# rlawhdrhs/Vision-Transformer-OpenCL

Hardware: AMD Instinct MI355X
Metric: images/sec ViT-B/16 224² fp32 @batch256; % MFMA roofline; top-1 match (higher is better)
Workload: dtype f32; 1 GPU; ViT-B/16 224x224 fp32 forward, batch 256 per GPU, synthetic weights and images (BASELINE.json configs[1]); batch_per_gpu=256, global_batch=256, parallelism=dp1, lanes_per_gpu=1, prune_last_layer=False, ln_fold=True, device=AMD Radeon Graphics, arch=gfx950:sramecc+:xnack-, compute_units=256, clock_mhz=2400

## Files before the change

### include/vit_hip_kernels.h

```cpp
#ifndef VIT_HIP_KERNELS_H
#define VIT_HIP_KERNELS_H

#include <stddef.h>

#ifdef __cplusplus
extern "C" {
#endif

typedef void *vithip_stream_t;
typedef void *vithip_event_t;
typedef void *vithip_graph_t;

typedef struct {
    char name[256];
    char arch[64];
    int compute_units;
    int clock_mhz;
    int wavefront;
    int lds_per_block;
    unsigned long long hbm_bytes;
} vithip_device_info;

const char *vithip_error_string(int code);
int vithip_device_count(int *count);
// ... 81 lines not shown
int vithip_gemm_bf16(vithip_stream_t stream, const vithip_gemm_bf16_args *args);
int vithip_ln_fold_weights(vithip_stream_t stream, const float *W, const float *bias, const float *gamma, const float *beta,
                           unsigned short *Wf, float *colsum, float *bias_f, int N, int K);
#define VITHIP_QSCALE 0.18033688011112042f
int vithip_ln_fold_weights_scaled(vithip_stream_t stream, const float *W, const float *bias, const float *gamma, const float *beta,
                                  unsigned short *Wf, float *colsum, float *bias_f, int N, int K, int scale_rows, float scale);
int vithip_rowstats_bf16(vithip_stream_t stream, const float *x, size_t ldx, unsigned short *x16, size_t ldx16,
                         float *rows_out, int rows, int dim);
int vithip_rowstats_bf16_eps(vithip_stream_t stream, const float *x, size_t ldx, unsigned short *x16, size_t ldx16,
                             float *rows_out, int rows, int dim, double eps);
int vithip_ln_strips(int N);
int vithip_rowstats_finalize(vithip_stream_t stream, const float *partials, int strips, int rows, int dim, float *rows_out);
int vithip_rowstats_finalize_eps(vithip_stream_t stream, const float *partials, int strips, int rows, int dim, float *rows_out, double eps);
int vithip_gather_rows_f32(vithip_stream_t stream, const float *src, size_t src_stride, float *dst, size_t dst_stride, int rows,
                           int width);
int vithip_layernorm_f32_bf16out(vithip_stream_t stream, const float *x, size_t ldx, unsigned short *y, size_t ldy,
                                 const float *gamma, const float *beta, int rows, int dim);
int vithip_layernorm_f32_bf16out_eps(vithip_stream_t stream, const float *x, size_t ldx, unsigned short *y, size_t ldy,
                                     const float *gamma, const float *beta, int rows, int dim, double eps);
int vithip_attention_bf16io(vithip_stream_t stream, const unsigned short *qkv, unsigned short *out,
                            int n_images, int tokens, int heads);
int vithip_attention_bf16io_f32math(vithip_stream_t stream, const unsigned short *qkv, unsigned short *out,
                                    int n_images, int tokens, int heads);
int vithip_attention_f32_rows(vithip_stream_t stream, const float *qkv, float *out, int n_images, int tokens, int heads,
                              int q_rows);
int vithip_attention_bf16io_rows(vithip_stream_t stream, const unsigned short *qkv, unsigned short *out, int n_images,
                                 int tokens, int heads, int q_rows);
int vithip_attention_bf16io_qscaled(vithip_stream_t stream, const unsigned short *qkv, unsigned short *out, int n_images,
                                    int tokens, int heads, int q_rows);
int vithip_attention_f32_hd(vithip_stream_t stream, const float *qkv, float *out, int n_images, int tokens, int heads, int head_dim,
                            int q_rows);
int vithip_attention_bf16io_hd(vithip_stream_t stream, const unsigned short *qkv, unsigned short *out, int n_images, int tokens,
                               int heads, int head_dim, int q_rows, int q_scaled);
float vithip_qscale(int head_dim);
int vithip_patch_embed_bf16(vithip_stream_t stream, const float *images, const unsigned short *conv_w16,
                            const float *conv_b, const float *cls, const float *pos, float *x,
                            unsigned short *patches16, int n_images, int img_size, int patch_size, int in_chans,
                            int embed_dim);
int vithip_patch_embed_bf16_implicit(vithip_stream_t stream, const float *images, const unsigned short *conv_w16,
                                     const float *conv_b, const float *cls, const float *pos, float *x,
                                     int n_images, int img_size, int patch_size, int in_chans, int embed_dim);
int vithip_f32_to_bf16(vithip_stream_t stream, const float *src, unsigned short *dst, size_t count);

int vithip_patch_embed_f32(vithip_stream_t stream, const float *images, const float *conv_w,
                           const float *conv_b, const float *cls, const float *pos, float *x,
                           int n_images, int img_size, int patch_size, int in_chans, int embed_dim);
int vithip_patch_embed_f32_general(vithip_stream_t stream, const float *images, const float *conv_w,
                                   const float *conv_b, const float *cls, const float *pos, float *x,
                                   int n_images, int img_size, int patch_size, int in_chans, int embed_dim);

int vithip_layernorm_f32(vithip_stream_t stream, const float *x, size_t ldx, float *y, size_t ldy,
                         const float *gamma, const float *beta, int rows, int dim);
int vithip_layernorm_f32_eps(vithip_stream_t stream, const float *x, size_t ldx, float *y, size_t ldy,
                             const float *gamma, const float *beta, int rows, int dim, double eps);

int vithip_swiglu_f32(vithip_stream_t stream, const float *u, size_t ldu, float *h, size_t ldh, int rows, int H);
int vithip_swiglu_bf16(vithip_stream_t stream, const unsigned short *u, size_t ldu, unsigned short *h, size_t ldh, int rows, int H);

int vithip_attention_f32(vithip_stream_t stream, const float *qkv, float *out,
                         int n_images, int tokens, int heads);

int vithip_softmax_top1_f32(vithip_stream_t stream, const float *logits, int ld_logits,
                            float *probs, int ld_probs, int *top1_label, float *top1_prob,
                            int rows, int classes);

enum { VITHIP_SCORE_PROB = 0, VITHIP_SCORE_LOGIT = 1 };
// ... 59 lines not shown
```

### vision-transformer-opencl_amd/binding.py

```python
from __future__ import annotations

import ctypes as C
import os
from typing import Optional, Sequence

import numpy as np

from .synth import MLP_CODES, MLP_SHIFT, ModelConfig

HERE = os.path.dirname(os.path.abspath(__file__))
LIB_PATH = os.environ.get("VIT_HIP_LIBRARY") or os.path.join(HERE, "libvit_mi355x.so")

f32p = C.POINTER(C.c_float)
i32p = C.POINTER(C.c_int)

STAGES = ("embed", "ln", "qkv", "attn", "outproj", "fc1", "fc2", "head", "softmax")
IMAGENET_MEAN = (0.485, 0.456, 0.406)
IMAGENET_STD = (0.229, 0.224, 0.225)
EPI_BIAS, EPI_BIAS_GELU, EPI_BIAS_RESIDUAL = 0, 1, 2
EPI_BIAS_QGELU = 6
ARITH_F32, ARITH_SPLIT3 = 0, 1


class VitError(RuntimeError):
# ... 305 lines not shown
        L.vit_argmax.argtypes = [f32p, C.c_int]
        L.ViT_hip.argtypes = [C.POINTER(CImageData), C.POINTER(CNetwork), C.POINTER(f32p)]
        L.ViT_opencl.argtypes = [C.POINTER(CImageData), C.POINTER(CNetwork), C.POINTER(f32p)]
        for fn in ("vithip_malloc", "vithip_host_alloc"):
            getattr(L, fn).argtypes = [C.POINTER(C.c_void_p), C.c_size_t]
        L.vithip_free.argtypes = [C.c_void_p]
        for fn in ("vithip_memcpy_h2d", "vithip_memcpy_d2h", "vithip_memcpy_d2d"):
            getattr(L, fn).argtypes = [C.c_void_p, C.c_void_p, C.c_size_t, C.c_void_p]
        L.vithip_gemm_f32.argtypes = [C.c_void_p, C.POINTER(CGemmArgs)]
        L.vithip_split3_weights_bytes.argtypes = [C.c_int, C.c_int]
        L.vithip_split3_weights_bytes.restype = C.c_size_t
        L.vithip_split3_weights_f32.argtypes = [C.c_void_p, C.c_void_p, C.c_int, C.c_int, C.c_int, C.c_void_p]
        L.vithip_patch_embed_f32.argtypes = [C.c_void_p] + [C.c_void_p] * 6 + [C.c_int] * 5
        if hasattr(L, "vithip_patch_embed_f32_general"):
            L.vithip_patch_embed_f32_general.argtypes = [C.c_void_p] + [C.c_void_p] * 6 + [C.c_int] * 5
            L.vit_weights_fold_layer_scale.argtypes = [C.POINTER(CConfig), C.POINTER(CNetwork), C.c_int, C.POINTER(CNetwork), C.c_int]
        L.vithip_layernorm_f32.argtypes = [C.c_void_p, C.c_void_p, C.c_size_t, C.c_void_p, C.c_size_t,
                                           C.c_void_p, C.c_void_p, C.c_int, C.c_int]
        pv, cls = [C.c_void_p] * 3, [C.c_void_p, C.c_void_p, C.c_size_t, C.c_void_p, C.c_size_t]
        for fn in ("vithip_attention_f32", "vithip_attention_bf16io", "vithip_attention_bf16io_f32math"):
            getattr(L, fn).argtypes = pv + [C.c_int] * 3
        for fn in ("vithip_attention_f32_rows", "vithip_attention_bf16io_rows", "vithip_attention_bf16io_qscaled"):
            getattr(L, fn).argtypes = pv + [C.c_int] * 4
        if hasattr(L, "vit_engine_cls_attention_device"):
            L.vithip_cls_attention_f32.argtypes = cls + [C.c_int] * 4
            L.vithip_cls_attention_bf16.argtypes = cls + [C.c_int] * 5
        if hasattr(L, "vithip_attention_f32_hd"):
            L.vithip_qscale.restype = C.c_float
            L.vithip_qscale.argtypes = [C.c_int]
            L.vithip_attention_f32_hd.argtypes = pv + [C.c_int] * 5
            L.vithip_attention_bf16io_hd.argtypes = pv + [C.c_int] * 6
            L.vithip_cls_attention_f32_hd.argtypes = cls + [C.c_int] * 5
            L.vithip_cls_attention_bf16_hd.argtypes = cls + [C.c_int] * 6
        L.vithip_softmax_top1_f32.argtypes = [C.c_void_p, C.c_void_p, C.c_int, C.c_void_p, C.c_int, C.c_void_p,
                                              C.c_void_p, C.c_int, C.c_int]
        L.vithip_event_create.argtypes = [C.POINTER(C.c_void_p)]
        L.vithip_event_record.argtypes = [C.c_void_p, C.c_void_p]
        L.vithip_event_sync.argtypes = [C.c_void_p]
        L.vithip_event_destroy.argtypes = [C.c_void_p]
        L.vithip_event_elapsed_ms.argtypes = [C.POINTER(C.c_float), C.c_void_p, C.c_void_p]
        L.vithip_stream_sync.argtypes = [C.c_void_p]
        L.vithip_get_device_info.argtypes = [C.c_int, C.POINTER(CDeviceInfo)]
        _lib = L
    return _lib


def hip_check(rc: int, what: str = "HIP call") -> None:
    if rc != 0:
        err = VitError(f"{what}: HIP error {rc} ({lib().vithip_error_string(rc).decode()})")
        err.code = int(rc)
        raise err


def _as_f32(a) -> np.ndarray:
    return np.ascontiguousarray(a, dtype=np.float32)


def networks_from(weights: Sequence[np.ndarray]):
    arr = (CNetwork * len(weights))()
    keep = []
    for i, w in enumerate(weights):
        if w is None:
            arr[i].data = None
            arr[i].size = 0
        else:
            w = _as_f32(w)
# ... 526 lines not shown
    _note(out, dst=dd)
    hip_check(L.vithip_gather_rows_f32(None, None if null == "src" else ds.ptr, ds.ld if src_stride is None else src_stride,
                                       None if null == "dst" else dd.ptr, dd.ld if dst_stride is None else dst_stride,
                                       src.shape[0] if rows is None else rows, src.shape[1] if width is None else width),
              "vithip_gather_rows_f32")
    return dd.window()


def attention(qkv, n_images: int, tokens: int, heads: int) -> np.ndarray:
    return _attention("vithip_attention_f32", _as_f32(qkv), n_images, tokens, heads, 64, ())


def attention_rows(qkv, n_images: int, tokens: int, heads: int, q_rows: int, fill: float = 0.0, frames=None,
                   out: Optional[dict] = None) -> np.ndarray:
    return _attention("vithip_attention_f32_rows", _as_f32(qkv), n_images, tokens, heads, 64, (q_rows,), fill, frames, out)


def attention_bf16io_rows(qkv_bits, n_images: int, tokens: int, heads: int, q_rows: int, q_scaled: bool = False, frames=None,
                          out: Optional[dict] = None) -> np.ndarray:
    name = "vithip_attention_bf16io_qscaled" if q_scaled else "vithip_attention_bf16io_rows"
    return _attention(name, _bits(qkv_bits), n_images, tokens, heads, 64, (q_rows,), 0, frames, out)


def qscale(head_dim: int) -> float:
    return float(lib().vithip_qscale(int(head_dim)))


def attention_hd(qkv, n_images: int, tokens: int, heads: int, head_dim: int, q_rows: Optional[int] = None, fill: float = 0.0,
                 frames=None, out: Optional[dict] = None) -> np.ndarray:
    return _attention("vithip_attention_f32_hd", _as_f32(qkv), n_images, tokens, heads, head_dim,
                      (head_dim, tokens if q_rows is None else q_rows), fill, frames, out)


def attention_bf16io_hd(qkv_bits, n_images: int, tokens: int, heads: int, head_dim: int, q_rows: Optional[int] = None,
                        q_scaled: bool = False, fill: int = 0, frames=None, out: Optional[dict] = None) -> np.ndarray:
    return _attention("vithip_attention_bf16io_hd", _bits(qkv_bits), n_images, tokens, heads, head_dim,
                      (head_dim, tokens if q_rows is None else q_rows, int(q_scaled)), fill, frames, out)


def _cls_attention(name, qkv, n_images, tokens, heads, head_dim, head_mean, q_scaled, ld_out, fill):
    assert qkv.shape == (n_images * tokens, 3 * heads * head_dim)
    args = ((head_dim,) if name.endswith("_hd") else ()) + (int(head_mean),) + (() if q_scaled is None else (int(q_scaled),))
    row = tokens if head_mean else heads * tokens
    ld = row if ld_out is None else int(ld_out)
    do = DeviceArray((n_images, ld)) if fill is None else DeviceArray.from_numpy(np.full((n_images, ld), fill, np.float32))
    dq = DeviceArray.from_numpy(qkv)
    hip_check(getattr(lib(), name)(None, dq.ptr, 3 * heads * head_dim, do.ptr, ld, n_images, tokens, heads, *args), name)
    res = do.numpy()
    if ld_out is not None:
        return res
    return res if head_mean else res.reshape(n_images, heads, tokens)


def cls_attention(qkv, n_images: int, tokens: int, heads: int, head_mean: bool = False, ld_out: Optional[int] = None,
                  fill: Optional[float] = None) -> np.ndarray:
    return _cls_attention("vithip_cls_attention_f32", _as_f32(qkv), n_images, tokens, heads, 64, head_mean, None, ld_out, fill)


def cls_attention_bf16(qkv_bits, n_images: int, tokens: int, heads: int, head_mean: bool = False, q_scaled: bool = False,
                       ld_out: Optional[int] = None, fill: Optional[float] = None) -> np.ndarray:
    return _cls_attention("vithip_cls_attention_bf16", _bits(qkv_bits), n_images, tokens, heads, 64, head_mean, q_scaled, ld_out, fill)


def cls_attention_hd(qkv, n_images: int, tokens: int, heads: int, head_dim: int, head_mean: bool = False, ld_out: Optional[int] = None,
                     fill: Optional[float] = None) -> np.ndarray:
    return _cls_attention("vithip_cls_attention_f32_hd", _as_f32(qkv), n_images, tokens, heads, head_dim, head_mean, None, ld_out, fill)
# ... 738 lines not shown
```

### vision-transformer-opencl_amd/csrc/vit_attention.hip

```cpp
#include <hip/hip_runtime.h>

#include <type_traits>

#include "vit_attention.hpp"
#include "vit_device.hpp"
#include "vit_hip_kernels.h"
#ifdef VIT_PROBES
#include "vit_probes.h"
#endif

namespace {

using namespace vitattn;

template <typename IO> __device__ __forceinline__ f32x4 load4(const IO *p);
template <> __device__ __forceinline__ f32x4 load4<float>(const float *p) { return *reinterpret_cast<const f32x4 *>(p); }
template <> __device__ __forceinline__ f32x4 load4<bf16_t>(const bf16_t *p) {
    const uint2 b = *reinterpret_cast<const uint2 *>(p);
    f32x4 v;
    v[0] = __uint_as_float(b.x << 16);
    v[1] = __uint_as_float(b.x & 0xffff0000u);
    v[2] = __uint_as_float(b.y << 16);
    v[3] = __uint_as_float(b.y & 0xffff0000u);
    return v;
// ... 667 lines not shown
    hipLaunchKernelGGL(attention_bf16_kernel<NKT>, dim3(grid), dim3(ATT_THREADS), 0, s, qkv, out, tokens, heads, items, q_rows,
                       q_scaled ? 1.0f : kScale64);
    return static_cast<int>(hipGetLastError());
}

template <int NKT, typename IO>
int launch_f32(hipStream_t s, const IO *qkv, IO *out, int n_images, int tokens, int heads, int q_rows) {
    hipLaunchKernelGGL((attention_f32_kernel<NKT, IO>), dim3(heads, n_images), dim3(ATT_THREADS), 0, s, qkv, out,
                       tokens, heads, q_rows, g_attn_dbg);
    return static_cast<int>(hipGetLastError());
}

inline dim3 chunked_grid(int n_images, int tokens, int heads) {
    return dim3(heads, n_images, ((tokens + 31) / 32 + ATT_WAVES - 1) / ATT_WAVES);
}

template <typename IO>
int route_f32_math(hipStream_t s, const IO *qkv, IO *out, int n_images, int tokens, int heads, int q_rows) {
    if constexpr (std::is_same<IO, float>::value) {
        if (tokens <= 224) return attention_f32_resident(s, qkv, out, n_images, tokens, heads, q_rows);
    }
    if (tokens > 224) {
        hipLaunchKernelGGL(attention_f32_chunked_kernel<IO>, chunked_grid(n_images, tokens, heads), dim3(ATT_THREADS), 0, s, qkv, out,
                           tokens, heads);
        return static_cast<int>(hipGetLastError());
    }
    return dispatch_int<1, 7>((tokens + 31) / 32, [&](auto nkt) {
        return launch_f32<decltype(nkt)::value, IO>(s, qkv, out, n_images, tokens, heads, q_rows);
    });
}

template <typename IO>
int route(vithip_stream_t stream, const IO *qkv, IO *out, int n_images, int tokens, int heads, int head_dim, int q_rows, int q_scaled,
          bool f32_math = false, bool resident_only = false) {
    constexpr int refused = static_cast<int>(hipErrorInvalidValue);
    hipStream_t s = static_cast<hipStream_t>(stream);
    if (!hd_accepted(head_dim) || (q_scaled != 0 && q_scaled != 1) || !qkv_args_ok(qkv, out, n_images, tokens, heads, q_rows))
        return refused;
    if constexpr (std::is_same<IO, float>::value) {
        if (head_dim != 64) return attention_hd_f32(s, qkv, out, n_images, tokens, heads, head_dim, q_rows);
        if (tokens > 224 && (resident_only || q_rows < tokens)) return refused;
        return route_f32_math<float>(s, qkv, out, n_images, tokens, heads, q_rows);
    } else {
        if (head_dim != 64) return attention_hd_bf16(s, qkv, out, n_images, tokens, heads, head_dim, q_rows, q_scaled != 0);
        if (tokens > 224 && (resident_only || q_rows < tokens)) return refused;
        if (f32_math) return q_scaled ? refused : route_f32_math<bf16_t>(s, qkv, out, n_images, tokens, heads, q_rows);
        if (tokens <= 224)
            return dispatch_int<1, 7>((tokens + 31) / 32, [&](auto nkt) {
                return launch_bf16<decltype(nkt)::value>(s, qkv, out, n_images, tokens, heads, q_rows, q_scaled != 0);
            });
        if (tokens <= 704) return attention_bf16_stream(s, qkv, out, n_images, tokens, heads, q_scaled != 0);
        hipLaunchKernelGGL(attention_bf16_chunked_kernel, chunked_grid(n_images, tokens, heads), dim3(ATT_THREADS), 0, s, qkv, out, tokens,
                           heads, q_scaled ? 1.0f : kScale64);
        return static_cast<int>(hipGetLastError());
    }
}

}

#ifdef VIT_PROBES
extern "C" int vithip_attention_set_probe_mode(int mode) {
    vitattn::g_res_mode = mode;
    return 0;
}
extern "C" int vithip_attention_set_debug_buffer(void *buf) {
    g_attn_dbg = static_cast<unsigned long long *>(buf);
    vitattn::g_res_dbg = g_attn_dbg;
    vitattn::g_stream_dbg = g_attn_dbg;
    return 0;
}
#endif

extern "C" {


int vithip_attention_f32(vithip_stream_t stream, const float *qkv, float *out, int n_images, int tokens, int heads) {
    return route<float>(stream, qkv, out, n_images, tokens, heads, 64, tokens, 0);
}

int vithip_attention_f32_rows(vithip_stream_t stream, const float *qkv, float *out, int n_images, int tokens, int heads, int q_rows) {
    return route<float>(stream, qkv, out, n_images, tokens, heads, 64, q_rows, 0, false, true);
}

int vithip_attention_f32_hd(vithip_stream_t stream, const float *qkv, float *out, int n_images, int tokens, int heads, int head_dim,
                            int q_rows) {
    return route<float>(stream, qkv, out, n_images, tokens, heads, head_dim, q_rows, 0);
}

int vithip_attention_bf16io(vithip_stream_t stream, const unsigned short *qkv, unsigned short *out, int n_images, int tokens,
                            int heads) {
    return route<bf16_t>(stream, qkv, out, n_images, tokens, heads, 64, tokens, 0);
}

int vithip_attention_bf16io_rows(vithip_stream_t stream, const unsigned short *qkv, unsigned short *out, int n_images, int tokens,
                                 int heads, int q_rows) {
    return route<bf16_t>(stream, qkv, out, n_images, tokens, heads, 64, q_rows, 0, false, true);
}

int vithip_attention_bf16io_qscaled(vithip_stream_t stream, const unsigned short *qkv, unsigned short *out, int n_images, int tokens,
                                    int heads, int q_rows) {
    return route<bf16_t>(stream, qkv, out, n_images, tokens, heads, 64, q_rows, 1);
}

int vithip_attention_bf16io_f32math(vithip_stream_t stream, const unsigned short *qkv, unsigned short *out, int n_images, int tokens,
                                    int heads) {
    return route<bf16_t>(stream, qkv, out, n_images, tokens, heads, 64, tokens, 0, true);
}

int vithip_attention_bf16io_hd(vithip_stream_t stream, const unsigned short *qkv, unsigned short *out, int n_images, int tokens,
                               int heads, int head_dim, int q_rows, int q_scaled) {
    return route<bf16_t>(stream, qkv, out, n_images, tokens, heads, head_dim, q_rows, q_scaled);
}

}
```

### vision-transformer-opencl_amd/csrc/vit_attention.hpp

```cpp
#ifndef VIT_ATTENTION_HPP
#define VIT_ATTENTION_HPP

#include <hip/hip_runtime.h>

#include <type_traits>

#include "vit_hip_kernels.h"

namespace vitattn {

typedef float f32x4 __attribute__((ext_vector_type(4)));
typedef float f32x16 __attribute__((ext_vector_type(16)));
typedef unsigned short bf16_t;
typedef __attribute__((ext_vector_type(4))) __bf16 bf16x4;
typedef __attribute__((ext_vector_type(8))) __bf16 bf16x8;
typedef unsigned u32x4 __attribute__((ext_vector_type(4)));
typedef short short4v __attribute__((ext_vector_type(4)));
typedef short short8v __attribute__((ext_vector_type(8)));
typedef __attribute__((address_space(3))) short4v lds_short4v;
typedef __attribute__((address_space(3))) void lds_void;

constexpr float kScale64 = 0.125f * 1.4426950408889634f;
static_assert(kScale64 == VITHIP_QSCALE, "the kernels' factor and the one the engine folds into the Q rows are the same bits");

// ... 4 lines not shown
    const int chunk = (dt * 4 + 2 * g2 + (pq >> 1)) ^ (4 * ((q >> 1) & 1));
    const bf16_t *ptr = Vs + row * LD + chunk * 8 + 4 * (pq & 1);
    const short4v lo = __builtin_amdgcn_ds_read_tr16_b64_v4i16((lds_short4v *)ptr);
    const short4v hi = __builtin_amdgcn_ds_read_tr16_b64_v4i16((lds_short4v *)(ptr + 8 * LD));
    const short8v both = __builtin_shufflevector(lo, hi, 0, 1, 2, 3, 4, 5, 6, 7);
    return __builtin_bit_cast(bf16x8, both);
}


static inline bool qkv_args_ok(const void *qkv, const void *out, int n_images, int tokens, int heads, int q_rows) {
    const size_t low_bits = (reinterpret_cast<size_t>(qkv) | reinterpret_cast<size_t>(out)) & 15;
    return qkv && out && !low_bits && n_images > 0 && tokens > 0 && heads > 0 && q_rows > 0 && q_rows <= tokens;
}

static inline bool hd_accepted(int head_dim) { return head_dim == 64 || (head_dim >= 72 && head_dim <= 128 && head_dim % 8 == 0); }

template <int FIRST, int COUNT, int STEP = 1, typename F>
static inline int dispatch_int(int n, F &&f) {
    if constexpr (COUNT == 0) {
        return static_cast<int>(hipErrorInvalidValue);
    } else {
        if (n == FIRST) return f(std::integral_constant<int, FIRST>{});
        return dispatch_int<FIRST + STEP, COUNT - 1, STEP>(n, f);
    }
}


int attention_f32_resident(hipStream_t s, const float *qkv, float *out, int n_images, int tokens, int heads, int q_rows);
int attention_bf16_stream(hipStream_t s, const unsigned short *qkv, unsigned short *out, int n_images, int tokens, int heads, bool q_scaled);
__attribute__((visibility("hidden"))) int attention_hd_f32(hipStream_t s, const float *qkv, float *out, int n_images, int tokens,
                                                           int heads, int head_dim, int q_rows);
__attribute__((visibility("hidden"))) int attention_hd_bf16(hipStream_t s, const unsigned short *qkv, unsigned short *out, int n_images,
                                                            int tokens, int heads, int head_dim, int q_rows, bool q_scaled);

#ifdef VIT_PROBES
extern unsigned long long *g_res_dbg;
extern int g_res_mode;
extern unsigned long long *g_stream_dbg;
#endif

}

#endif
```

### vision-transformer-opencl_amd/csrc/vit_attention_hd.hip

```cpp
#include <hip/hip_runtime.h>

#include <math.h>

#include <type_traits>

#include "vit_attention.hpp"
#include "vit_hip_kernels.h"

namespace {

using namespace vitattn;
typedef unsigned int u32x2 __attribute__((ext_vector_type(2)));

constexpr int HD_WAVES = 4, HD_THREADS = HD_WAVES * 64;
constexpr int HD_QROWS = HD_WAVES * 32;

template <int HD, bool BF16>
struct Geo {
    typedef typename std::conditional<BF16, bf16_t, float>::type elem;
    static constexpr int VEC = BF16 ? 8 : 4;
    static constexpr int KC = BF16 ? 64 : 32;
    static constexpr int KT = KC / 32;
    static constexpr int DT = (HD + 31) / 32;
    static constexpr int HDK = BF16 ? (HD + 15) / 16 * 16 : HD;
    static constexpr int KROW = HDK + (BF16 ? 8 : 4);
    static constexpr int VROW = KC + 4;
    static constexpr int K_ELEMS = KC * KROW, V_ELEMS = DT * 32 * VROW;
    static constexpr int MIN_WAVES = BF16 && HD <= 96 ? 4 : 3;
};

template <int HD, bool BF16, bool QS>
__global__ __launch_bounds__(HD_THREADS, (Geo<HD, BF16>::MIN_WAVES)) void attention_hd_kernel(
    const typename Geo<HD, BF16>::elem *__restrict__ qkv, typename Geo<HD, BF16>::elem *__restrict__ out, int tokens, int heads, int q_rows,
    int qblocks, float scale) {
    typedef Geo<HD, BF16> G;
    typedef typename G::elem elem;
    constexpr int VEC = G::VEC, KC = G::KC, KT = G::KT, DT = G::DT, KROW = G::KROW, VROW = G::VROW;
    __shared__ __attribute__((aligned(16))) elem Ks[G::K_ELEMS];
    __shared__ __attribute__((aligned(16))) elem Vt[G::V_ELEMS];

// ... 144 lines not shown
#pragma unroll
                            for (int i = 0; i < 4; ++i) o[dt] = __builtin_amdgcn_mfma_f32_32x32x2f32(vf[i], s[4 * q + i], o[dt], 0, 0, 0);
                        }
                }
            }
        }
        __syncthreads();
    }

    const int qrow = qrow0 + r;
    if (active && qrow < q_rows) {
        const float inv = 1.0f / (l_run + __shfl_xor(l_run, 32));
        elem *dst = out + ((size_t)image * tokens + qrow) * D + (size_t)head * HD;
#pragma unroll
        for (int dt = 0; dt < DT; ++dt)
#pragma unroll
            for (int q = 0; q < 4; ++q) {
                const int d0 = 32 * dt + 8 * q + 4 * h;
                if (d0 < HD) {
                    if constexpr (BF16) {
                        bf16x4 w;
#pragma unroll
                        for (int i = 0; i < 4; ++i) w[i] = (__bf16)(o[dt][4 * q + i] * inv);
                        *reinterpret_cast<u32x2 *>(dst + d0) = __builtin_bit_cast(u32x2, w);
                    } else {
                        const f32x4 w = {o[dt][4 * q] * inv, o[dt][4 * q + 1] * inv, o[dt][4 * q + 2] * inv, o[dt][4 * q + 3] * inv};
                        *reinterpret_cast<f32x4 *>(dst + d0) = w;
                    }
                }
            }
    }
}

template <bool BF16, bool QS>
int launch_hd(hipStream_t s, const typename Geo<128, BF16>::elem *qkv, typename Geo<128, BF16>::elem *out, int n_images, int tokens,
              int heads, int head_dim, int q_rows) {
    const int qblocks = (q_rows + HD_QROWS - 1) / HD_QROWS;
    if (heads > 65535 || (long long)n_images * qblocks > 0x7fffffffLL) return static_cast<int>(hipErrorInvalidValue);
    const float scale = QS ? 1.0f : vithip_qscale(head_dim);
    return dispatch_int<72, 8, 8>(head_dim, [&](auto hd) {
        hipLaunchKernelGGL((attention_hd_kernel<decltype(hd)::value, BF16, QS>), dim3((unsigned)(n_images * qblocks), (unsigned)heads),
                           dim3(HD_THREADS), 0, s, qkv, out, tokens, heads, q_rows, qblocks, scale);
        return static_cast<int>(hipGetLastError());
    });
}

}

int vitattn::attention_hd_f32(hipStream_t s, const float *qkv, float *out, int n_images, int tokens, int heads, int head_dim, int q_rows) {
    return launch_hd<false, false>(s, qkv, out, n_images, tokens, heads, head_dim, q_rows);
}

int vitattn::attention_hd_bf16(hipStream_t s, const unsigned short *qkv, unsigned short *out, int n_images, int tokens, int heads,
                               int head_dim, int q_rows, bool q_scaled) {
    return q_scaled ? launch_hd<true, true>(s, qkv, out, n_images, tokens, heads, head_dim, q_rows)
                    : launch_hd<true, false>(s, qkv, out, n_images, tokens, heads, head_dim, q_rows);
}

extern "C" float vithip_qscale(int head_dim) {
    if (!vitattn::hd_accepted(head_dim)) return 0.0f;
    return (float)((1.0 / sqrt((double)head_dim)) * 1.4426950408889634074);
}
```

### vision-transformer-opencl_amd/csrc/vit_gemm_common.hpp

```cpp
#pragma once
#include <hip/hip_runtime.h>

#include <type_traits>

#include "vit_hip_kernels.h"

namespace vitgemm {


typedef float f32x16 __attribute__((ext_vector_type(16)));
typedef float f32x4 __attribute__((ext_vector_type(4)));
typedef float f32x2 __attribute__((ext_vector_type(2)));
typedef unsigned u32x4 __attribute__((ext_vector_type(4)));

constexpr int KALIGN = 32;

enum { A_DENSE = 0, A_PATCHES = 1 };
enum { EPI_BIAS_LN = 3, EPI_BIAS_GELU_LN = 4, EPI_RESIDUAL_STATS = 5, EPI_BIAS_QGELU_LN = 7  };
constexpr bool epi_is_fold(int epi) { return epi == EPI_BIAS_LN || epi == EPI_BIAS_GELU_LN || epi == EPI_BIAS_QGELU_LN; }
constexpr bool epi_is_gelu(int epi) { return epi == VITHIP_EPI_BIAS_GELU || epi == EPI_BIAS_GELU_LN; }
constexpr bool epi_is_qgelu(int epi) { return epi == VITHIP_EPI_BIAS_QGELU || epi == EPI_BIAS_QGELU_LN; }

struct GemmParams {
    const float *A;
    const float *W;
    const float *bias;
    const float *R;
    float *C;
    int lda, ldw, ldr, ldc;
    int M, N, K;
    int tiles_m, tiles_n;
    int group_m;
    const float *pos;
    unsigned long long *dbg;
    int patches;
    int grid;
    int patch;
    int img;
// ... 130 lines not shown
}
__device__ __forceinline__ void quick_gelu_x8(float (&y)[8]) {
    f32x2 yy[4];
#pragma unroll
    for (int v = 0; v < 4; ++v) yy[v] = f32x2{y[2 * v], y[2 * v + 1]};
    quick_gelu_lockstep<4>(yy);
#pragma unroll
    for (int v = 0; v < 4; ++v) y[2 * v] = yy[v].x, y[2 * v + 1] = yy[v].y;
}

__device__ __forceinline__ int xcd_remap(int bid, int nwg) {
    const int q = nwg >> 3, rem = nwg & 7;
    const int xcd = bid & 7, idx = bid >> 3;
    const int base = xcd < rem ? xcd * (q + 1) : rem * (q + 1) + (xcd - rem) * q;
    return base + idx;
}

__device__ __forceinline__ void tile_coords(int tile, int tiles_m, int tiles_n, int group_m, int &tm, int &tn) {
    const int per_group = group_m * tiles_n;
    const int g = tile / per_group, in_g = tile - g * per_group;
    const int first = g * group_m;
    const int rows = tiles_m - first < group_m ? tiles_m - first : group_m;
    tn = in_g / rows;
    tm = first + (in_g - tn * rows);
}


enum { ARITH_F32 = 0, ARITH_SPLIT3 = 1 };
typedef __bf16 bf16x8 __attribute__((ext_vector_type(8)));
typedef __bf16 bf16x4 __attribute__((ext_vector_type(4)));
typedef unsigned u32x2 __attribute__((ext_vector_type(2)));
constexpr int SPLIT_BK = 16;
constexpr int SPLIT_LD = 28;
constexpr int SPLIT_TERM_A[6] = {0, 2, 1, 0, 1, 0};
constexpr int SPLIT_TERM_W[6] = {2, 0, 1, 1, 0, 0};

__device__ __forceinline__ float bf16_to_f32(__bf16 v) {
    return __builtin_bit_cast(float, (unsigned)__builtin_bit_cast(unsigned short, v) << 16);
}
__device__ __forceinline__ u32x2 split3_piece(f32x4 &x, int piece) {
    bf16x4 b;
#pragma unroll
    for (int e = 0; e < 4; ++e) b[e] = (__bf16)x[e];
    if (piece < 2) {
#pragma unroll
        for (int e = 0; e < 4; ++e) x[e] = x[e] - bf16_to_f32(b[e]);
    }
    return __builtin_bit_cast(u32x2, b);
}
__device__ __forceinline__ void split3_store(float *row, int kc, f32x4 x) {
#pragma unroll
    for (int piece = 0; piece < 3; ++piece) *reinterpret_cast<u32x2 *>(row + piece * 8 + kc / 2) = split3_piece(x, piece);
}
__device__ __forceinline__ u32x4 split3_piece8(f32x4 &x0, f32x4 &x1, int piece) {
    const u32x2 p0 = split3_piece(x0, piece), p1 = split3_piece(x1, piece);
    return u32x4{p0[0], p0[1], p1[0], p1[1]};
}

__device__ __forceinline__ unsigned split3_piece2(f32x2 &x, int piece) {
    typedef __bf16 bf16x2 __attribute__((ext_vector_type(2)));
    bf16x2 b;
#pragma unroll
    for (int e = 0; e < 2; ++e) b[e] = (__bf16)x[e];
    if (piece < 2) x = x - f32x2{bf16_to_f32(b[0]), bf16_to_f32(b[1])};
    return __builtin_bit_cast(unsigned, b);
}

constexpr int WIMG_ROWS = 128;
constexpr int WIMG_BLOCK_BYTES = 3 * WIMG_ROWS * SPLIT_BK * 2;
constexpr int SPLIT_LD_SW = 32;
__device__ __forceinline__ int split_swizzle(int row) { return 2 * ((row & 3) ^ ((row >> 2) & 3)) + ((row >> 3) & 1); }
__device__ __forceinline__ int split_sw_offset(int row, int s) { return row * SPLIT_LD_SW + 4 * (s ^ split_swizzle(row)); }
template <int TM, int TN, int NS, typename Restage>
__device__ __forceinline__ void split3_step(f32x16 (&acc)[TM][TN], const float *As, const float *Bs, Restage &&restage) {
    bf16x8 a[TM][3], b[TN][3];
#pragma unroll
    for (int o = 0; o < 3; ++o) {
        const int pa = SPLIT_TERM_A[o], pb = SPLIT_TERM_W[o];
#pragma unroll
        for (int i = 0; i < TM; ++i) a[i][pa] = *reinterpret_cast<const bf16x8 *>(As + i * 32 * SPLIT_LD + pa * 8);
#pragma unroll
        for (int j = 0; j < TN; ++j) b[j][pb] = *reinterpret_cast<const bf16x8 *>(Bs + j * 32 * SPLIT_LD + pb * 8);
    }
    __builtin_amdgcn_sched_barrier(0);
    constexpr int NM = 6 * TM * TN, NR = NM / 2 > 0 ? NM / 2 : 1;
#pragma unroll
    for (int idx = 0; idx < NM; ++idx) {
        const int t = idx / (TM * TN), i = (idx / TN) % TM, j = idx % TN;
        acc[i][j] = __builtin_amdgcn_mfma_f32_32x32x16_bf16(a[i][SPLIT_TERM_A[t]], b[j][SPLIT_TERM_W[t]], acc[i][j], 0, 0, 0);
        if (idx < NR) {
            const int slot_before = (idx * NS) / NR, slot_after = ((idx + 1) * NS) / NR;
            if (slot_after > slot_before) {
                __builtin_amdgcn_sched_barrier(0);
#pragma unroll
                for (int q = slot_before; q < slot_after; ++q) restage(q);
                __builtin_amdgcn_sched_barrier(0);
            }
        }
// ... 434 lines not shown
```

### vision-transformer-opencl_amd/host/vit_engine.c

```c
#include "vit_engine.h"

#include <limits.h>
#include <math.h>
#include <stdarg.h>
#include <stddef.h>
#include <stdio.h>
#include <stdlib.h>
#include <omp.h>
#include <string.h>

#include "vit_hip_kernels.h"
#include "vit_io.h"

#define VIT_MAX_LANES 4
#define MAX_EVENTS 4096
#define VIT_MAX_U8_CHANS 4

enum { VIT_IN_F32 = 0, VIT_IN_U8 = 1, VIT_IN_IMAGES = 2 };
typedef struct {
    int kind;
    int resize_shorter;
    int resize_filter;
    float mean[VIT_MAX_U8_CHANS], std[VIT_MAX_U8_CHANS];
} vit_input;
// ... 867 lines not shown
    for (int j = 0; j < c->L; ++j) {
        rows[j] = pruned ? c->lane[j].n : c->lane[j].n * T;
        pairs[j] = pruned ? c->lane[j].cls_pairs : c->lane[j].tok_pairs;
    }

    for (int j = 0; j < c->L; ++j) {
        vit_lane *ln = &c->lane[j];
        if (!fold) RUN(layernorm(c, ln->s, ln->x, D, ln->y, D, o->ln1_g, o->ln1_b, ln->n * T));
        else if (!ln->stats_ready) RUN(row_stats(c, ln, D, ln->tok_pairs, ln->n * T));
    }
    for (int j = 0; j < c->L; ++j) {
        vit_lane *ln = &c->lane[j];
        gemm_desc g = {.stage = VIT_STAGE_QKV, .bf16 = bf16, .A = fold ? ln->xa : ln->y, .lda = D, .ops = o->qkv, .C = ln->qkv,
                       .ldc = 3 * D, .M = ln->n * T, .N = 3 * D, .K = D, .role = VITHIP_EPI_BIAS, .ln_rows = ln->tok_pairs};
        if (pruned) {
            gemm_desc kv = g;
            kv.ops.W = at(g.ops.W, (size_t)D * D, c->esz); kv.ops.bias = g.ops.bias + D; kv.C = at(ln->qkv, D, c->esz); kv.N = 2 * D;
            kv.ops.colsum = g.ops.colsum ? g.ops.colsum + D : NULL;
            kv.ops.w_split = g.ops.w_split && D % 128 == 0 ? at(g.ops.w_split, (size_t)D * D * 6, 1) : NULL;
            RUN(gemm(e, ln->s, &kv, NULL));
            if (fold) {
                HIP_TRY(e, stage_begin(e, ln->s, VIT_STAGE_LN));
                HIP_TRY(e, vithip_gather_rows_f32(ln->s, ln->tok_pairs, (size_t)2 * T, ln->cls_pairs, 2, ln->n, 2));
                HIP_TRY(e, stage_end(e, ln->s));
            }
            g.lda = r * D; g.ldc = r * 3 * D; g.M = rows[j]; g.N = D; g.ln_rows = pairs[j];
        }
        RUN(gemm(e, ln->s, &g, NULL));
    }
    if (c->qkv_only && !feeds_next) return VIT_OK;
    for (int j = 0; j < c->L; ++j) {
        const vit_lane *ln = &c->lane[j];
        HIP_TRY(e, stage_begin(e, ln->s, VIT_STAGE_ATTN));
        if (!bf16) HIP_TRY(e, vithip_attention_f32_hd(ln->s, ln->qkv, ln->y, ln->n, T, heads, D / heads, pruned ? 1 : T));
        else HIP_TRY(e, vithip_attention_bf16io_hd(ln->s, ln->qkv, ln->y, ln->n, T, heads, D / heads, pruned ? 1 : T, fold));
        HIP_TRY(e, stage_end(e, ln->s));
    }
    for (int j = 0; j < c->L; ++j) {
        vit_lane *ln = &c->lane[j];
        gemm_desc g = {.stage = VIT_STAGE_OUTPROJ, .bf16 = bf16, .A = ln->y, .lda = r * D, .ops = o->out, .C = ln->x,
                       .ldc = r * D, .M = rows[j], .N = D, .K = D, .role = VITHIP_EPI_BIAS_RESIDUAL};
        if (fold && (bf16 || !pruned)) { g.stats_rows = pairs[j]; g.stats_part = ln->partials; g.x16 = bf16 ? ln->xa : NULL; }
        RUN(gemm(e, ln->s, &g, &ln2_ready[j]));
    }
    for (int j = 0; j < c->L; ++j) {
        const vit_lane *ln = &c->lane[j];
        if (!fold) RUN(layernorm(c, ln->s, ln->x, (size_t)r * D, ln->y, D, o->ln2_g, o->ln2_b, rows[j]));
        else if (!ln2_ready[j]) RUN(row_stats(c, ln, (size_t)r * D, pairs[j], rows[j]));
    }
    for (int j = 0; j < c->L; ++j) {
        const vit_lane *ln = &c->lane[j];
        gemm_desc g = {.stage = VIT_STAGE_FC1, .bf16 = bf16, .A = ln->y, .lda = D, .ops = o->fc1, .C = ln->h, .ldc = H1,
                       .M = rows[j], .N = H1, .K = D, .role = fc1_role};
        if (fold) { g.A = ln->xa; g.lda = r * D; g.ln_rows = pairs[j]; }
        RUN(gemm(e, ln->s, &g, NULL));
        if (swiglu) {
            HIP_TRY(e, stage_begin(e, ln->s, VIT_STAGE_FC1));
            if (bf16) HIP_TRY(e, vithip_swiglu_bf16(ln->s, ln->h, (size_t)H1, ln->h, (size_t)H1, rows[j], H));
            else HIP_TRY(e, vithip_swiglu_f32(ln->s, ln->h, (size_t)H1, ln->h, (size_t)H1, rows[j], H));
            HIP_TRY(e, stage_end(e, ln->s));
        }
    }
    for (int j = 0; j < c->L; ++j) {
        vit_lane *ln = &c->lane[j];
        gemm_desc g = {.stage = VIT_STAGE_FC2, .bf16 = bf16, .A = ln->h, .lda = H1, .ops = o->fc2, .C = ln->x, .ldc = r * D,
                       .M = rows[j], .N = D, .K = H, .role = VITHIP_EPI_BIAS_RESIDUAL};
        if (fold && feeds_next) { g.stats_rows = ln->tok_pairs; g.stats_part = ln->partials; g.x16 = bf16 ? ln->xa : NULL; }
// ... 1035 lines not shown
```

Before: 5538 images/sec.

## Add split-bf16x3 MFMA flash attention kernel for fp32 head_dim 64

Adds an fp32 attention kernel that splits Q, K, V and P into three bf16 pieces and runs six bf16 MFMA product terms per tile, emulating fp32 accuracy on matrix cores. It uses an online softmax with deferred rescaling, and stages K and a transposed V in LDS per key chunk. The engine routes fp32 attention to it when split arithmetic is enabled and head_dim is 64. This aims to replace slower fp32 attention math with MFMA throughput, at the cost of six times the MFMA work per product, extra register pressure, and small precision differences.

```diff
diff --git a/include/vit_hip_kernels.h b/include/vit_hip_kernels.h
--- a/include/vit_hip_kernels.h
+++ b/include/vit_hip_kernels.h
@@ -137,6 +137,8 @@
                             int q_rows);
 int vithip_attention_bf16io_hd(vithip_stream_t stream, const unsigned short *qkv, unsigned short *out, int n_images, int tokens,
                                int heads, int head_dim, int q_rows, int q_scaled);
+int vithip_attention_f32_split(vithip_stream_t stream, const float *qkv, float *out, int n_images, int tokens, int heads, int head_dim,
+                               int q_rows);
 float vithip_qscale(int head_dim);
 int vithip_patch_embed_bf16(vithip_stream_t stream, const float *images, const unsigned short *conv_w16,
                             const float *conv_b, const float *cls, const float *pos, float *x,
diff --git a/vision-transformer-opencl_amd/binding.py b/vision-transformer-opencl_amd/binding.py
--- a/vision-transformer-opencl_amd/binding.py
+++ b/vision-transformer-opencl_amd/binding.py
@@ -361,6 +361,8 @@
             L.vithip_attention_bf16io_hd.argtypes = pv + [C.c_int] * 6
             L.vithip_cls_attention_f32_hd.argtypes = cls + [C.c_int] * 5
             L.vithip_cls_attention_bf16_hd.argtypes = cls + [C.c_int] * 6
+        if hasattr(L, "vithip_attention_f32_split"):
+            L.vithip_attention_f32_split.argtypes = pv + [C.c_int] * 5
         L.vithip_softmax_top1_f32.argtypes = [C.c_void_p, C.c_void_p, C.c_int, C.c_void_p, C.c_int, C.c_void_p,
                                               C.c_void_p, C.c_int, C.c_int]
         L.vithip_event_create.argtypes = [C.POINTER(C.c_void_p)]
@@ -953,6 +955,12 @@
                       (head_dim, tokens if q_rows is None else q_rows), fill, frames, out)
 
 
+def attention_split(qkv, n_images: int, tokens: int, heads: int, q_rows: Optional[int] = None, fill: float = 0.0, frames=None,
+                    out: Optional[dict] = None) -> np.ndarray:
+    return _attention("vithip_attention_f32_split", _as_f32(qkv), n_images, tokens, heads, 64,
+                      (64, tokens if q_rows is None else q_rows), fill, frames, out)
+
+
 def attention_bf16io_hd(qkv_bits, n_images: int, tokens: int, heads: int, head_dim: int, q_rows: Optional[int] = None,
                         q_scaled: bool = False, fill: int = 0, frames=None, out: Optional[dict] = None) -> np.ndarray:
     return _attention("vithip_attention_bf16io_hd", _bits(qkv_bits), n_images, tokens, heads, head_dim,
diff --git a/vision-transformer-opencl_amd/csrc/vit_attention.hip b/vision-transformer-opencl_amd/csrc/vit_attention.hip
--- a/vision-transformer-opencl_amd/csrc/vit_attention.hip
+++ b/vision-transformer-opencl_amd/csrc/vit_attention.hip
@@ -723,12 +723,13 @@
 
 template <typename IO>
 int route(vithip_stream_t stream, const IO *qkv, IO *out, int n_images, int tokens, int heads, int head_dim, int q_rows, int q_scaled,
-          bool f32_math = false, bool resident_only = false) {
+          bool f32_math = false, bool resident_only = false, bool split = false) {
     constexpr int refused = static_cast<int>(hipErrorInvalidValue);
     hipStream_t s = static_cast<hipStream_t>(stream);
     if (!hd_accepted(head_dim) || (q_scaled != 0 && q_scaled != 1) || !qkv_args_ok(qkv, out, n_images, tokens, heads, q_rows))
         return refused;
     if constexpr (std::is_same<IO, float>::value) {
+        if (split) return head_dim == 64 ? attention_split_f32(s, qkv, out, n_images, tokens, heads, q_rows) : refused;
         if (head_dim != 64) return attention_hd_f32(s, qkv, out, n_images, tokens, heads, head_dim, q_rows);
         if (tokens > 224 && (resident_only || q_rows < tokens)) return refused;
         return route_f32_math<float>(s, qkv, out, n_images, tokens, heads, q_rows);
@@ -778,6 +779,11 @@
     return route<float>(stream, qkv, out, n_images, tokens, heads, head_dim, q_rows, 0);
 }
 
+int vithip_attention_f32_split(vithip_stream_t stream, const float *qkv, float *out, int n_images, int tokens, int heads, int head_dim,
+                               int q_rows) {
+    return route<float>(stream, qkv, out, n_images, tokens, heads, head_dim, q_rows, 0, false, false, true);
+}
+
 int vithip_attention_bf16io(vithip_stream_t stream, const unsigned short *qkv, unsigned short *out, int n_images, int tokens,
                             int heads) {
     return route<bf16_t>(stream, qkv, out, n_images, tokens, heads, 64, tokens, 0);
diff --git a/vision-transformer-opencl_amd/csrc/vit_attention.hpp b/vision-transformer-opencl_amd/csrc/vit_attention.hpp
--- a/vision-transformer-opencl_amd/csrc/vit_attention.hpp
+++ b/vision-transformer-opencl_amd/csrc/vit_attention.hpp
@@ -60,6 +60,8 @@
                                                            int heads, int head_dim, int q_rows);
 __attribute__((visibility("hidden"))) int attention_hd_bf16(hipStream_t s, const unsigned short *qkv, unsigned short *out, int n_images,
                                                             int tokens, int heads, int head_dim, int q_rows, bool q_scaled);
+__attribute__((visibility("hidden"))) int attention_split_f32(hipStream_t s, const float *qkv, float *out, int n_images, int tokens,
+                                                              int heads, int q_rows);
 
 #ifdef VIT_PROBES
 extern unsigned long long *g_res_dbg;
diff --git a/vision-transformer-opencl_amd/csrc/vit_attention_hd.hip b/vision-transformer-opencl_amd/csrc/vit_attention_hd.hip
--- a/vision-transformer-opencl_amd/csrc/vit_attention_hd.hip
+++ b/vision-transformer-opencl_amd/csrc/vit_attention_hd.hip
@@ -6,6 +6,7 @@
 
 #include "vit_attention.hpp"
 #include "vit_hip_kernels.h"
+#include "vit_split3.hpp"
 
 namespace {
 
@@ -216,6 +217,212 @@
     }
 }
 
+#ifndef ATT_SPLIT_WAVES
+#define ATT_SPLIT_WAVES 4
+#endif
+#ifndef ATT_SPLIT_MINW
+#define ATT_SPLIT_MINW 3
+#endif
+constexpr int SP_WAVES = ATT_SPLIT_WAVES, SP_THREADS = SP_WAVES * 64, SP_QROWS = SP_WAVES * 32;
+
+__global__ __launch_bounds__(SP_THREADS, ATT_SPLIT_MINW) void attention_split_kernel(const float *__restrict__ qkv, float *__restrict__ out,
+                                                                                    int tokens, int heads, int q_rows, int qblocks) {
+    using vitsplit::SPLIT_TERM_A;
+    using vitsplit::SPLIT_TERM_W;
+    using vitsplit::split3_piece8;
+    typedef Geo<64, true> G;
+    constexpr int HD = 64, KC = G::KC, KT = G::KT, DT = G::DT, KROW = G::KROW, VROW = G::VROW, NQ = HD / 16;
+    __shared__ __attribute__((aligned(16))) bf16_t Ks[3 * G::K_ELEMS];
+    __shared__ __attribute__((aligned(16))) bf16_t Vt[3 * G::V_ELEMS];
+
+    const int tid = threadIdx.x, lane = tid & 63, wave = tid >> 6;
+    const int r = lane & 31, h = lane >> 5;
+    const int image = blockIdx.x / qblocks, qblock = blockIdx.x - image * qblocks, head = blockIdx.y;
+    const size_t D = (size_t)heads * HD, ld = 3 * D;
+    const float *rows = qkv + (size_t)image * tokens * ld + (size_t)head * HD;
+    const float *krows = rows + D, *vrows = rows + 2 * D;
+    const int qrow0 = qblock * SP_QROWS + wave * 32;
+    const bool active = qrow0 < q_rows;
+    const f32x4 zero4 = {0.0f, 0.0f, 0.0f, 0.0f};
+
+    bf16x8 qf[3][NQ];
+    {
+        int qrow = qrow0 + r;
+        qrow = qrow < q_rows ? qrow : q_rows - 1;
+        const float *qp = rows + (size_t)qrow * ld + 8 * h;
+#pragma unroll
+        for (int ks = 0; ks < NQ; ++ks) {
+            f32x4 x0 = zero4, x1 = zero4;
+            if (active) {
+                x0 = *reinterpret_cast<const f32x4 *>(qp + 16 * ks);
+                x1 = *reinterpret_cast<const f32x4 *>(qp + 16 * ks + 4);
+            }
+#pragma unroll
+            for (int pl = 0; pl < 3; ++pl) qf[pl][ks] = __builtin_bit_cast(bf16x8, split3_piece8(x0, x1, pl));
+        }
+    }
+
+    f32x16 o[DT];
+#pragma unroll
+    for (int dt = 0; dt < DT; ++dt)
+#pragma unroll
+        for (int v = 0; v < 16; ++v) o[dt][v] = 0.0f;
+    float m_run = -INFINITY, l_run = 0.0f;
+
+    constexpr int K_ITEMS = KC * (HD / 8), V_ITEMS = (KC / 2) * (HD / 8);
+    constexpr int KI = (K_ITEMS + SP_THREADS - 1) / SP_THREADS;
+    constexpr int V_TID0 = SP_THREADS > V_ITEMS ? SP_THREADS - V_ITEMS : 0;
+    static_assert(V_ITEMS <= SP_THREADS, "one V item per thread at most");
+    const int vi = tid - V_TID0;
+    f32x4 kx[KI][2], vx[4];
+    auto fetch = [&](int key0) {
+#pragma unroll
+        for (int it = 0; it < KI; ++it) {
+            const int i = tid + it * SP_THREADS, row = i / (HD / 8), c = i - row * (HD / 8), key = key0 + row;
+            kx[it][0] = kx[it][1] = zero4;
+            if (i < K_ITEMS && key < tokens) {
+                const float *p = krows + (size_t)key * ld + 8 * c;
+                kx[it][0] = *reinterpret_cast<const f32x4 *>(p);
+                kx[it][1] = *reinterpret_cast<const f32x4 *>(p + 4);
+            }
+        }
+        if (vi >= 0) {
+            const int c = vi / (KC / 2), key = key0 + 2 * (vi - c * (KC / 2));
+#pragma unroll
+            for (int j = 0; j < 4; ++j) vx[j] = zero4;
+            if (key < tokens) {
+                const float *p = vrows + (size_t)key * ld + 8 * c;
+                vx[0] = *reinterpret_cast<const f32x4 *>(p);
+                vx[1] = *reinterpret_cast<const f32x4 *>(p + 4);
+            }
+            if (key + 1 < tokens) {
+                const float *p = vrows + (size_t)(key + 1) * ld + 8 * c;
+                vx[2] = *reinterpret_cast<const f32x4 *>(p);
+                vx[3] = *reinterpret_cast<const f32x4 *>(p + 4);
+            }
+        }
+    };
+    auto store = [&](bf16_t *Kd, bf16_t *Vd) {
+#pragma unroll
+        for (int it = 0; it < KI; ++it) {
+            const int i = tid + it * SP_THREADS, row = i / (HD / 8), c = i - row * (HD / 8);
+            if (i < K_ITEMS) {
+#pragma unroll
+                for (int pl = 0; pl < 3; ++pl)
+                    *reinterpret_cast<u32x4 *>(Kd + pl * G::K_ELEMS + row * KROW + 8 * c) = split3_piece8(kx[it][0], kx[it][1], pl);
+            }
+        }
+        if (vi >= 0) {
+            const int c = vi / (KC / 2), row = 2 * (vi - c * (KC / 2));
+#pragma unroll
+            for (int pl = 0; pl < 3; ++pl) {
+                const u32x4 a = split3_piece8(vx[0], vx[1], pl), b = split3_piece8(vx[2], vx[3], pl);
+                bf16_t *vd = Vd + pl * G::V_ELEMS + (c * 8) * VROW + row;
+#pragma unroll
+                for (int j = 0; j < 4; ++j) {
+                    *reinterpret_cast<unsigned *>(vd + (2 * j) * VROW) = (a[j] & 0xffffu) | (b[j] << 16);
+                    *reinterpret_cast<unsigned *>(vd + (2 * j + 1) * VROW) = (a[j] >> 16) | (b[j] & 0xffff0000u);
+                }
+            }
+        }
+    };
+
+    for (int key0 = 0; key0 < tokens; key0 += KC) {
+        fetch(key0);
+        store(Ks, Vt);
+        __syncthreads();
+
+        if (active) {
+#pragma unroll
+            for (int t = 0; t < KT; ++t) {
+                const int tile0 = key0 + 32 * t;
+                if (tile0 >= tokens) break;
+                f32x16 s;
+#pragma unroll
+                for (int v = 0; v < 16; ++v) s[v] = 0.0f;
+                const bf16_t *kp = Ks + (32 * t + r) * KROW + 8 * h;
+#pragma unroll
+                for (int ks = 0; ks < NQ; ++ks) {
+                    bf16x8 kf[3];
+#pragma unroll
+                    for (int pl = 0; pl < 3; ++pl) kf[pl] = *reinterpret_cast<const bf16x8 *>(kp + pl * G::K_ELEMS + 16 * ks);
+#pragma unroll
+                    for (int term = 0; term < 6; ++term)
+                        s = __builtin_amdgcn_mfma_f32_32x32x16_bf16(kf[SPLIT_TERM_A[term]], qf[SPLIT_TERM_W[term]][ks], s, 0, 0, 0);
+                }
+                if (tile0 + 32 > tokens) {
+#pragma unroll
+                    for (int v = 0; v < 16; ++v) {
+                        const int key = tile0 + (v & 3) + 8 * (v >> 2) + 4 * h;
+                        s[v] = key < tokens ? s[v] : -INFINITY;
+                    }
+                }
+                float cmax = s[0];
+#pragma unroll
+                for (int v = 1; v < 16; ++v) cmax = fmaxf(cmax, s[v]);
+                cmax = fmaxf(cmax, __shfl_xor(cmax, 32));
+                constexpr float kDefer = 8.0f, scale = kScale64;
+                const float m_old = m_run;
+                const float m_new = (cmax - m_old) * scale > kDefer ? cmax : m_old;
+                const float mneg = -m_new * scale;
+                m_run = m_new;
+                float sum = 0.0f;
+#pragma unroll
+                for (int v = 0; v < 16; ++v) {
+                    s[v] = __builtin_amdgcn_exp2f(fmaf(s[v], scale, mneg));
+                    sum += s[v];
+                }
+                if (__any(m_new != m_old)) {
+                    const float alpha = __builtin_amdgcn_exp2f((m_old - m_new) * scale);
+                    l_run *= alpha;
+#pragma unroll
+                    for (int dt = 0; dt < DT; ++dt)
+#pragma unroll
+                        for (int v = 0; v < 16; ++v) o[dt][v] *= alpha;
+                }
+                l_run += sum;
+#pragma unroll
+                for (int s2 = 0; s2 < 2; ++s2) {
+                    if (tile0 + 16 * s2 >= tokens) break;
+                    f32x4 x0 = {s[8 * s2], s[8 * s2 + 1], s[8 * s2 + 2], s[8 * s2 + 3]};
+                    f32x4 x1 = {s[8 * s2 + 4], s[8 * s2 + 5], s[8 * s2 + 6], s[8 * s2 + 7]};
+                    bf16x8 pf[3], vf[DT][3];
+#pragma unroll
+                    for (int pl = 0; pl < 3; ++pl) pf[pl] = __builtin_bit_cast(bf16x8, split3_piece8(x0, x1, pl));
+#pragma unroll
+                    for (int dt = 0; dt < DT; ++dt)
+#pragma unroll
+                        for (int pl = 0; pl < 3; ++pl) {
+                            const bf16_t *vp = Vt + pl * G::V_ELEMS + (32 * dt + r) * VROW + 32 * t + 16 * s2 + 4 * h;
+                            const u32x2 lo = *reinterpret_cast<const u32x2 *>(vp), hi = *reinterpret_cast<const u32x2 *>(vp + 8);
+                            const u32x4 both = {lo[0], lo[1], hi[0], hi[1]};
+                            vf[dt][pl] = __builtin_bit_cast(bf16x8, both);
+                        }
+#pragma unroll
+                    for (int term = 0; term < 6; ++term)
+#pragma unroll
+                        for (int dt = 0; dt < DT; ++dt)
+                            o[dt] = __builtin_amdgcn_mfma_f32_32x32x16_bf16(vf[dt][SPLIT_TERM_A[term]], pf[SPLIT_TERM_W[term]], o[dt], 0, 0, 0);
+                }
+            }
+        }
+        __syncthreads();
+    }
+
+    const int qrow = qrow0 + r;
+    if (active && qrow < q_rows) {
+        const float inv = 1.0f / (l_run + __shfl_xor(l_run, 32));
+        float *dst = out + ((size_t)image * tokens + qrow) * D + (size_t)head * HD + 4 * h;
+#pragma unroll
+        for (int dt = 0; dt < DT; ++dt)
+#pragma unroll
+            for (int q = 0; q < 4; ++q) {
+                const f32x4 w = {o[dt][4 * q] * inv, o[dt][4 * q + 1] * inv, o[dt][4 * q + 2] * inv, o[dt][4 * q + 3] * inv};
+                *reinterpret_cast<f32x4 *>(dst + 32 * dt + 8 * q) = w;
+            }
+    }
+}
+
 template <bool BF16, bool QS>
 int launch_hd(hipStream_t s, const typename Geo<128, BF16>::elem *qkv, typename Geo<128, BF16>::elem *out, int n_images, int tokens,
               int heads, int head_dim, int q_rows) {
@@ -241,6 +448,14 @@
                     : launch_hd<true, false>(s, qkv, out, n_images, tokens, heads, head_dim, q_rows);
 }
 
+int vitattn::attention_split_f32(hipStream_t s, const float *qkv, float *out, int n_images, int tokens, int heads, int q_rows) {
+    const int qblocks = (q_rows + SP_QROWS - 1) / SP_QROWS;
+    if (heads > 65535 || (long long)n_images * qblocks > 0x7fffffffLL) return static_cast<int>(hipErrorInvalidValue);
+    hipLaunchKernelGGL(attention_split_kernel, dim3((unsigned)(n_images * qblocks), (unsigned)heads), dim3(SP_THREADS), 0, s, qkv, out,
+                       tokens, heads, q_rows, qblocks);
+    return static_cast<int>(hipGetLastError());
+}
+
 extern "C" float vithip_qscale(int head_dim) {
     if (!vitattn::hd_accepted(head_dim)) return 0.0f;
     return (float)((1.0 / sqrt((double)head_dim)) * 1.4426950408889634074);
diff --git a/vision-transformer-opencl_amd/csrc/vit_gemm_common.hpp b/vision-transformer-opencl_amd/csrc/vit_gemm_common.hpp
--- a/vision-transformer-opencl_amd/csrc/vit_gemm_common.hpp
+++ b/vision-transformer-opencl_amd/csrc/vit_gemm_common.hpp
@@ -4,6 +4,7 @@
 #include <type_traits>
 
 #include "vit_hip_kernels.h"
+#include "vit_split3.hpp"
 
 namespace vitgemm {
 
@@ -200,38 +201,15 @@
 typedef unsigned u32x2 __attribute__((ext_vector_type(2)));
 constexpr int SPLIT_BK = 16;
 constexpr int SPLIT_LD = 28;
-constexpr int SPLIT_TERM_A[6] = {0, 2, 1, 0, 1, 0};
-constexpr int SPLIT_TERM_W[6] = {2, 0, 1, 1, 0, 0};
-
-__device__ __forceinline__ float bf16_to_f32(__bf16 v) {
-    return __builtin_bit_cast(float, (unsigned)__builtin_bit_cast(unsigned short, v) << 16);
-}
-__device__ __forceinline__ u32x2 split3_piece(f32x4 &x, int piece) {
-    bf16x4 b;
-#pragma unroll
-    for (int e = 0; e < 4; ++e) b[e] = (__bf16)x[e];
-    if (piece < 2) {
-#pragma unroll
-        for (int e = 0; e < 4; ++e) x[e] = x[e] - bf16_to_f32(b[e]);
-    }
-    return __builtin_bit_cast(u32x2, b);
-}
+using vitsplit::SPLIT_TERM_A;
+using vitsplit::SPLIT_TERM_W;
+using vitsplit::bf16_to_f32;
+using vitsplit::split3_piece;
+using vitsplit::split3_piece2;
+using vitsplit::split3_piece8;
 __device__ __forceinline__ void split3_store(float *row, int kc, f32x4 x) {
 #pragma unroll
     for (int piece = 0; piece < 3; ++piece) *reinterpret_cast<u32x2 *>(row + piece * 8 + kc / 2) = split3_piece(x, piece);
-}
-__device__ __forceinline__ u32x4 split3_piece8(f32x4 &x0, f32x4 &x1, int piece) {
-    const u32x2 p0 = split3_piece(x0, piece), p1 = split3_piece(x1, piece);
-    return u32x4{p0[0], p0[1], p1[0], p1[1]};
-}
-
-__device__ __forceinline__ unsigned split3_piece2(f32x2 &x, int piece) {
-    typedef __bf16 bf16x2 __attribute__((ext_vector_type(2)));
-    bf16x2 b;
-#pragma unroll
-    for (int e = 0; e < 2; ++e) b[e] = (__bf16)x[e];
-    if (piece < 2) x = x - f32x2{bf16_to_f32(b[0]), bf16_to_f32(b[1])};
-    return __builtin_bit_cast(unsigned, b);
 }
 
 constexpr int WIMG_ROWS = 128;
diff --git a/vision-transformer-opencl_amd/csrc/vit_split3.hpp b/vision-transformer-opencl_amd/csrc/vit_split3.hpp
--- /dev/null
+++ b/vision-transformer-opencl_amd/csrc/vit_split3.hpp
@@ -0,0 +1,42 @@
+#pragma once
+#include <hip/hip_runtime.h>
+
+namespace vitsplit {
+
+typedef float f32x4 __attribute__((ext_vector_type(4)));
+typedef float f32x2 __attribute__((ext_vector_type(2)));
+typedef unsigned u32x4 __attribute__((ext_vector_type(4)));
+typedef unsigned u32x2 __attribute__((ext_vector_type(2)));
+typedef __bf16 bf16x8 __attribute__((ext_vector_type(8)));
+typedef __bf16 bf16x4 __attribute__((ext_vector_type(4)));
+
+constexpr int SPLIT_TERM_A[6] = {0, 2, 1, 0, 1, 0};
+constexpr int SPLIT_TERM_W[6] = {2, 0, 1, 1, 0, 0};
+
+__device__ __forceinline__ float bf16_to_f32(__bf16 v) {
+    return __builtin_bit_cast(float, (unsigned)__builtin_bit_cast(unsigned short, v) << 16);
+}
+__device__ __forceinline__ u32x2 split3_piece(f32x4 &x, int piece) {
+    bf16x4 b;
+#pragma unroll
+    for (int e = 0; e < 4; ++e) b[e] = (__bf16)x[e];
+    if (piece < 2) {
+#pragma unroll
+        for (int e = 0; e < 4; ++e) x[e] = x[e] - bf16_to_f32(b[e]);
+    }
+    return __builtin_bit_cast(u32x2, b);
+}
+__device__ __forceinline__ u32x4 split3_piece8(f32x4 &x0, f32x4 &x1, int piece) {
+    const u32x2 p0 = split3_piece(x0, piece), p1 = split3_piece(x1, piece);
+    return u32x4{p0[0], p0[1], p1[0], p1[1]};
+}
+__device__ __forceinline__ unsigned split3_piece2(f32x2 &x, int piece) {
+    typedef __bf16 bf16x2 __attribute__((ext_vector_type(2)));
+    bf16x2 b;
+#pragma unroll
+    for (int e = 0; e < 2; ++e) b[e] = (__bf16)x[e];
+    if (piece < 2) x = x - f32x2{bf16_to_f32(b[0]), bf16_to_f32(b[1])};
+    return __builtin_bit_cast(unsigned, b);
+}
+
+}
diff --git a/vision-transformer-opencl_amd/host/vit_engine.c b/vision-transformer-opencl_amd/host/vit_engine.c
--- a/vision-transformer-opencl_amd/host/vit_engine.c
+++ b/vision-transformer-opencl_amd/host/vit_engine.c
@@ -923,7 +923,9 @@
     for (int j = 0; j < c->L; ++j) {
         const vit_lane *ln = &c->lane[j];
         HIP_TRY(e, stage_begin(e, ln->s, VIT_STAGE_ATTN));
-        if (!bf16) HIP_TRY(e, vithip_attention_f32_hd(ln->s, ln->qkv, ln->y, ln->n, T, heads, D / heads, pruned ? 1 : T));
+        if (!bf16 && e->split && D / heads == 64)
+            HIP_TRY(e, vithip_attention_f32_split(ln->s, ln->qkv, ln->y, ln->n, T, heads, 64, pruned ? 1 : T));
+        else if (!bf16) HIP_TRY(e, vithip_attention_f32_hd(ln->s, ln->qkv, ln->y, ln->n, T, heads, D / heads, pruned ? 1 : T));
         else HIP_TRY(e, vithip_attention_bf16io_hd(ln->s, ln->qkv, ln->y, ln->n, T, heads, D / heads, pruned ? 1 : T, fold));
         HIP_TRY(e, stage_end(e, ln->s));
     }
```

Measured after the change: 5595 images/sec, median of 6. +1.0%, better.
